# Circuitscape/Circuitscape.jl

Hardware: NVIDIA H100
Metric: pair_solves_per_sec (higher is better)
Workload: dtype f64

## Files before the change

### circuitscape_b200/csrc/cs_b200.cu

```cuda
#include "../../include/cs_b200.h"

#include <cuda_runtime.h>
#include <cub/device/device_radix_sort.cuh>
#include <cub/device/device_scan.cuh>
#include <cub/device/device_select.cuh>

#include <algorithm>
#include <chrono>
#include <cmath>
#include <cstdarg>
#include <cstdio>
#include <cstdlib>
#include <cstring>
#include <limits>
#include <string>
#include <type_traits>
#include <vector>

#include "amg_host.hpp"
#include "win_host.hpp"
#include "kernels.cuh"
#include "raster_assembly.cuh"
#include "setup_device.hpp"

using namespace csb;

namespace {

thread_local std::string g_create_error;

constexpr int PROF_CLASSES = 20;
constexpr int PROF_PJ = 7;
constexpr int PROF_CGF = 8;
constexpr int PROF_RSW = 9;

struct GraphSlot {
  cudaGraphExec_t exec = nullptr;
  int chunk = 0;
  int64_t kernels = 0, spmms = 0;
  cudaGraphExec_t loop_exec = nullptr;
  int64_t loop_kernels = 0, loop_spmms = 0;
};

}

struct DevCsr {
  int* rowptr = nullptr;
  int* colidx = nullptr;
  void* vals = nullptr;
  int* bstart = nullptr;
  int nblocks = 0;
  int nrows = 0;
  int64_t nnz = 0;
  int lpr = 1;
  WinMeta* win_meta = nullptr;
  unsigned char* blob = nullptr;
  int has_dinv = 0;
  int64_t win_blocks = 0;
  int win_nblocks = 0;
  void* dia = nullptr;
  size_t dia_ld = 0;
  int dia_nr = 0;
  int dia_half = 0;
  int* ell_col = nullptr;
  void* ell_val = nullptr;
  size_t ell_ld = 0;
};

struct DevLevel {
  int64_t n = 0, n_pad = 0;
  DevCsr A, P, R;
  void* dinv = nullptr;
  double omega = 2.0 / 3.0;
  void *x = nullptr, *b = nullptr, *t = nullptr, *y = nullptr;
};

struct cs_b200_handle {
  int device = 0;
  int dtype = CS_B200_F64;
  int64_t n = 0, n_pad = 0, nnz = 0;
  int* d_rowptr = nullptr;
  int* d_colidx = nullptr;
  void* d_vals = nullptr;
  bool owns_matrix = true;
  void* d_vals0 = nullptr;
  void* d_fg = nullptr;
  void* d_plan = nullptr;
  int64_t plan_ncol = 0, plan_nset = 0, plan_nsrc = 0;
  void* d_dinv = nullptr;
  int* d_bstart = nullptr;
  int nblocks = 0;
  int ktmax = 8;
  void *X = nullptr, *R = nullptr, *P = nullptr, *AP = nullptr, *B = nullptr, *stage = nullptr;
  void* Z = nullptr;
  void* P2 = nullptr;
  void* R2 = nullptr;
  DevCsr A0;
  std::vector<DevLevel> lv;
  double* d_pinv = nullptr;
  double amg_opc = 0.0;
  bool amg = false;
  bool mixed = false;
  std::vector<DevLevel> lv32;
  void *R32 = nullptr, *X32 = nullptr, *T32 = nullptr, *Z32 = nullptr;
  void *d_cum = nullptr, *d_max = nullptr;
  int* d_bptr = nullptr;
  int64_t nb = 0;
  void* d_cum_branch = nullptr;
  void* d_branch_stage = nullptr;
  PanelCtl* d_ctl = nullptr;
  PanelCtl* h_ctl = nullptr;
  double* d_partials = nullptr;
  float* d_flush = nullptr;
  size_t flush_elems = 0;
  cudaStream_t stream = nullptr;
  cudaEvent_t ev0 = nullptr, ev1 = nullptr, ev2 = nullptr, ev3 = nullptr;
  long long* d_sp_rows = nullptr;
// ... 1229 lines not shown
template <typename F>
decltype(auto) with_width(int kt, F&& f) {
  DISPATCH_KT(kt, return f(std::integral_constant<int, KT>{}));
}

template <typename F>
decltype(auto) with_type_width(const cs_b200_handle* h, int kt, F&& f) {
  return with_type(h, [&](auto t) -> decltype(auto) {
    return with_width(kt, [&](auto KT) -> decltype(auto) { return f(t, KT); });
  });
}

struct ColumnDriver {
  cs_b200_handle* h;
  bool any_fail = false, any_maxit = false;
  std::string msg;

  template <typename Panel>
  int run(int64_t c_begin, int64_t c_end, Panel&& panel) {
    for (int64_t c0 = c_begin; c0 < c_end;) {
      const int kt = next_kt(c_end - c0, h->ktmax);
      if (int rc = with_width(kt, [&](auto KT) { return panel(KT, c0); })) return rc;
      c0 += kt;
    }
    return CS_B200_OK;
  }

  template <typename T, int KT>
  int solve(int64_t c0, double rtol, int64_t itmax, int64_t* iters, double* relres, bool masked = false) {
    h->rg_on = masked;
    const int rc = solve_panel<T, KT>(h, rtol, itmax);
    h->rg_on = false;
    h->pair_b = false;
    if (!rc) gather(KT, c0, iters, relres, itmax);
    return rc;
  }

  void gather(int kt, int64_t c0, int64_t* iters, double* relres, int64_t itmax) {
    for (int c = 0; c < kt; ++c) {
      const PanelCtl& ct = *h->h_ctl;
      const double bn = ct.bnorm[c];
      const double rr = bn > 0 ? std::sqrt(ct.resid[c] / bn) : 0.0;
      if (iters) iters[c0 + c] = ct.iters[c];
      if (relres) relres[c0 + c] = rr;
      h->stats.iterations += ct.iters[c];
      if (!(rr < h->opts.resid_gate)) {
        if (!any_fail) {
          char buf[256];
          snprintf(buf, sizeof buf,
                   "CUDA PCG solver residual %g exceeds tolerance %g for column %lld (%d iterations)",
                   rr, h->opts.resid_gate, (long long)(c0 + c + 1), ct.iters[c]);
          msg = buf;
        }
        any_fail = true;
      }
      if ((ct.iters[c] >= itmax || ct.stalled[c]) && std::sqrt(ct.rho[c]) > ct.tol[c]) any_maxit = true;
    }
  }

  int verdict(int rc) const {
    if (rc) return rc;
    if (any_fail) return set_err(h, CS_B200_ERR_RESIDUAL, "%s", msg.c_str());
    if (any_maxit) return set_err(h, CS_B200_ERR_MAXITER, "itmax reached (or the recurrence stagnated) before rtol");
    return CS_B200_OK;
  }
};

template <int KT>
int cur_grid(cs_b200_handle* h) {
  return (int)std::min<int64_t>(h->grid_spmm, (h->n + (NT / KT) - 1) / (NT / KT));
}

template <typename T, int KT>
void launch_cur_max(cs_b200_handle* h) {
  const int grid = cur_grid<KT>(h);
  if (h->A0.dia)
    k_cur_max_dia<T, KT><<<grid, NT, 0, h->stream>>>(dia_view<T>(h->A0), (const T*)h->X, h->d_ctl, h->d_partials);
  else
    k_cur_max<T, KT><<<grid, NT, 0, h->stream>>>((int)h->n, h->d_rowptr, h->d_colidx, (const T*)h->d_vals,
                                                 (const T*)h->X, h->d_ctl, h->d_partials);
  h->stats.kernel_launches++;
}

template <typename T, int KT>
void launch_currents(cs_b200_handle* h, bool want_curr, int accumulate, const void* fg = nullptr) {
  const int grid = cur_grid<KT>(h);
  launch_cur_max<T, KT>(h);
  if (h->A0.dia) {
    const DiaDev<T> a = dia_view<T>(h->A0);
    k_cur_acc_dia<T, KT><<<grid, NT, 0, h->stream>>>(a, (const T*)h->X, (const T*)fg, h->d_ctl,
                                                     want_curr ? (T*)h->AP : nullptr,
                                                     (T*)h->d_cum, (T*)h->d_max, accumulate, h->opts.log_transform, KT);
  } else {
    k_cur_acc<T, KT><<<grid, NT, 0, h->stream>>>((int)h->n, h->d_rowptr, h->d_colidx, (const T*)h->d_vals,
                                                 (const T*)h->X, (const T*)fg, h->d_ctl,
                                                 want_curr ? (T*)h->AP : nullptr,
                                                 (T*)h->d_cum, (T*)h->d_max, accumulate, h->opts.log_transform, KT);
  }
  h->stats.kernel_launches++;
}

struct ColCtl {
  long long src, dst;
  double weight;
};

inline double col_weight(const double* weight, int64_t c) { return weight ? weight[c] : 1.0; }

template <typename Col>
int upload_ctl(cs_b200_handle* h, int kt, Col&& col) {
  PanelCtl* hc = h->h_ctl;
  std::memset(hc, 0, sizeof(PanelCtl));
  for (int c = 0; c < kt; ++c) {
    const ColCtl v = col(c);
    hc->src[c] = v.src;
    hc->dst[c] = v.dst;
    hc->weight[c] = v.weight;
  }
  CK(h, cudaMemcpyAsync(h->d_ctl, hc, sizeof(PanelCtl), cudaMemcpyHostToDevice, h->stream));
  h->stats.h2d_bytes += sizeof(PanelCtl);
  return CS_B200_OK;
}

int read_ctl(cs_b200_handle* h) {
  CK(h, cudaMemcpyAsync(h->h_ctl, h->d_ctl, sizeof(PanelCtl), cudaMemcpyDeviceToHost, h->stream));
  CK(h, cudaStreamSynchronize(h->stream));
  h->stats.d2h_bytes += sizeof(PanelCtl);
  return CS_B200_OK;
}

int upload_sparse_rhs(cs_b200_handle* h, int kt, const int64_t* ptr, const int64_t* rows, const double* vals) {
  int ent_ptr[MAXKT + 1];
  for (int c = 0; c <= kt; ++c) ent_ptr[c] = (int)(ptr[c] - ptr[0]);
  const size_t nent = (size_t)ent_ptr[kt];
  if (!h->d_sp_ptr || nent > h->sp_cap) {
    cudaFree(h->d_sp_ptr); cudaFree(h->d_sp_rows); cudaFree(h->d_sp_vals);
    h->d_sp_ptr = nullptr; h->d_sp_rows = nullptr; h->d_sp_vals = nullptr;
    h->sp_cap = 0;
    const size_t cap = std::max<size_t>(nent, 1024);
    CK(h, cudaMalloc(&h->d_sp_ptr, (MAXKT + 1) * sizeof(int)));
    CK(h, cudaMalloc(&h->d_sp_rows, cap * sizeof(long long)));
    CK(h, cudaMalloc(&h->d_sp_vals, cap * sizeof(double)));
    h->sp_cap = cap;
  }
  CK(h, h2d(h, h->d_sp_ptr, ent_ptr, (kt + 1) * sizeof(int)));
  CK(h, h2d(h, h->d_sp_rows, rows + ptr[0], nent * sizeof(long long)));
  CK(h, h2d(h, h->d_sp_vals, vals + ptr[0], nent * sizeof(double)));
  h->stats.h2d_bytes += (kt + 1) * sizeof(int) + nent * 16.0;
  return CS_B200_OK;
}

int upload_set_segments(cs_b200_handle* h, int kt, const int64_t* set_ptr, const int64_t* set_rows,
                        const int64_t* set_a, const int64_t* set_b) {
  int seg[2 * MAXKT + 1];
  std::vector<int> rows;
  seg[0] = 0;
  for (int s = 0; s < 2 * kt; ++s) {
    const int64_t* sets = (s & 1) ? set_b : set_a;
    if (sets && sets[s / 2] >= 0)
      for (int64_t e = set_ptr[sets[s / 2]]; e < set_ptr[sets[s / 2] + 1]; ++e) rows.push_back((int)set_rows[e]);
    seg[s + 1] = (int)rows.size();
  }
  if (!h->d_rg_seg || rows.size() > h->rg_cap) {
    CK(h, cudaStreamSynchronize(h->stream));
    drop_graphs(h->rgraphs);
    cudaFree(h->d_rg_seg); cudaFree(h->d_rg_rows);
    h->d_rg_seg = nullptr; h->d_rg_rows = nullptr;
    h->rg_cap = 0;
    const size_t cap = std::max<size_t>(rows.size(), 4096);
    CK(h, cudaMalloc(&h->d_rg_seg, (2 * MAXKT + 1) * sizeof(int)));
// ... 2034 lines not shown
```

### circuitscape_b200/csrc/kernels.cuh

```cuda
#pragma once
#include <cuda_runtime.h>
#include <stdint.h>

namespace csb {

constexpr int NT = 256;
constexpr int NWARP = NT / 32;
constexpr int NNZ_CAP = 2304;
constexpr int MAXKT = 8;

struct PanelCtl {
  double rho[MAXKT];
  double pap[MAXKT];
  double alpha[MAXKT];
  double beta[MAXKT];
  double tol[MAXKT];
  double rho0[MAXKT];
  double resid[MAXKT];
  double bnorm[MAXKT];
  double xsrc[MAXKT];
  double xdst[MAXKT];
  double maxpos[MAXKT];
  double maxneg[MAXKT];
  double weight[MAXKT];
// ... 2216 lines not shown
  const int c = threadIdx.x;
  if (c < KT) {
    const long long s = ctl->src[c], d = ctl->dst[c];
    if (s >= 0 && d >= 0 && s != d) {
      B[(size_t)s * KT + c] = T(-1);
      B[(size_t)d * KT + c] = T(1);
    }
  }
}

template <typename T, int KT>
__global__ void k_pair_extract(const T* X, PanelCtl* ctl) {
  const int c = threadIdx.x;
  if (c < KT) {
    const long long s = ctl->src[c], d = ctl->dst[c];
    ctl->xsrc[c] = s >= 0 ? (double)X[(size_t)s * KT + c] : 0.0;
    ctl->xdst[c] = d >= 0 ? (double)X[(size_t)d * KT + c] : 0.0;
  }
}

template <typename T, int KT>
__global__ void k_sparse_rhs(T* B, const int* __restrict__ ent_ptr, const long long* __restrict__ rows,
                             const double* __restrict__ vals) {
  const int c = threadIdx.x;
  if (c < KT)
    for (int e = ent_ptr[c]; e < ent_ptr[c + 1]; ++e) B[(size_t)rows[e] * KT + c] += (T)vals[e];
}

template <typename T, int KT>
__global__ void k_probe(const T* __restrict__ X, const PanelCtl* __restrict__ ctl,
                        const long long* __restrict__ probe, int nprobe, T* __restrict__ out) {
  for (int e = blockIdx.x * blockDim.x + threadIdx.x; e < nprobe * KT; e += gridDim.x * blockDim.x) {
    const int c = e / nprobe, i = e % nprobe;
    out[e] = (T)((double)X[(size_t)probe[i] * KT + c] - ctl->xsrc[c]);
  }
}

template <typename T, int KT>
__global__ void k_combine(int n, size_t n_pad, const T* __restrict__ U, const int* __restrict__ ci,
                          const int* __restrict__ cj, T* __restrict__ X) {
  const size_t total = n_pad * KT;
  for (size_t e = (size_t)blockIdx.x * blockDim.x + threadIdx.x; e < total; e += (size_t)gridDim.x * blockDim.x) {
    const size_t i = e / KT;
    const int c = (int)(e % KT);
    T v = T(0);
    if (i < (size_t)n) {
      const int a = ci[c], b = cj[c];
      v = (b >= 0 ? U[(size_t)b * n_pad + i] : T(0)) - (a >= 0 ? U[(size_t)a * n_pad + i] : T(0));
    }
    X[e] = v;
  }
}

template <typename T, int KT>
__global__ void k_cm_to_panel(int n, size_t ld, const T* __restrict__ cm, T* __restrict__ panel,
                              int ncols) {
  const size_t total = (size_t)n * KT;
  for (size_t e = (size_t)blockIdx.x * blockDim.x + threadIdx.x; e < total;
       e += (size_t)gridDim.x * blockDim.x) {
    const size_t i = e / KT;
    const int c = (int)(e % KT);
    panel[e] = c < ncols ? cm[(size_t)c * ld + i] : T(0);
  }
}
template <typename T, int KT>
__global__ void k_panel_to_cm(int n, size_t ld, const T* __restrict__ panel, T* __restrict__ cm,
                              const PanelCtl* ctl, int use_shift) {
  const size_t total = (size_t)n * KT;
  for (size_t e = (size_t)blockIdx.x * blockDim.x + threadIdx.x; e < total;
       e += (size_t)gridDim.x * blockDim.x) {
    const size_t i = e / KT;
    const int c = (int)(e % KT);
    const T sh = use_shift ? (T)ctl->xsrc[c] : T(0);
    cm[(size_t)c * ld + i] = panel[e] - sh;
  }
}

template <typename T>
__device__ __forceinline__ void ground_current(T x, T& inflow, T& outflow) {
  if (x < T(0)) inflow -= x;
  if (x > T(0)) outflow += x;
}

template <typename T, int KT>
__global__ void __launch_bounds__(NT)
k_cur_max(int n, const int* __restrict__ rowptr, const int* __restrict__ colidx,
          const T* __restrict__ vals, const T* __restrict__ V, PanelCtl* ctl, double* partials) {
  CSB_REDUCE_SMEM(2, KT)
  const int c = threadIdx.x % KT;
  constexpr int RPP = NT / KT;
  double mp = -1.0e300, mn = -1.0e300;
  for (int row = blockIdx.x * RPP + threadIdx.x / KT; row < n; row += gridDim.x * RPP) {
    const T vi = V[(size_t)row * KT + c];
    for (int j = rowptr[row]; j < rowptr[row + 1]; ++j) {
      const int col = colidx[j];
      if (col > row) {
        const T d = fabs(vals[j]) * (vi - V[(size_t)col * KT + c]);
        mp = fmax(mp, (double)d);
        mn = fmax(mn, (double)(-d));
      }
    }
  }
  double v[2][1] = {{mp}, {mn}};
  if (grid_reduce<KT, 1, 2, true>(v, partials, &ctl->ticket, s_warp, s_tree, s_out)) {
    if (threadIdx.x < KT) {
      ctl->maxpos[threadIdx.x] = s_out[threadIdx.x];
      ctl->maxneg[threadIdx.x] = s_out[KT + threadIdx.x];
    }
  }
}

template <typename T, int KT>
__global__ void __launch_bounds__(NT)
k_cur_acc(int n, const int* __restrict__ rowptr, const int* __restrict__ colidx,
          const T* __restrict__ vals, const T* __restrict__ V, const T* __restrict__ fg, const PanelCtl* ctl,
          T* __restrict__ cur_out , T* __restrict__ cum, T* __restrict__ mx,
          int accumulate, int log_transform, int ncols) {
  const int c = threadIdx.x % KT;
  constexpr int RPP = NT / KT;
  const T maxpos = (T)ctl->maxpos[c], maxneg = (T)ctl->maxneg[c];
  const double w = ctl->weight[c];
  const int nrow_iter = (n + RPP - 1) / RPP;
  for (int it = blockIdx.x; it < nrow_iter; it += gridDim.x) {
    const int row = it * RPP + threadIdx.x / KT;
    T cur = T(0);
    if (row < n) {
      const T vi = V[(size_t)row * KT + c];
      T inflow = T(0), outflow = T(0);
      for (int j = rowptr[row]; j < rowptr[row + 1]; ++j) {
        const int col = colidx[j];
        if (col == row) continue;
        const T d = fabs(vals[j]) * (vi - V[(size_t)col * KT + c]);
        if (!(fabs(d / maxneg) < T(1e-8)) && d > T(0)) outflow += d;
        if (!(fabs(d / maxpos) < T(1e-8)) && d < T(0)) inflow -= d;
      }
      if (fg) ground_current(fg[row] * vi, inflow, outflow);
      cur = inflow > outflow ? inflow : outflow;
      if (cur_out) cur_out[(size_t)row * KT + c] = cur;
    }
    if (accumulate) {
      T val = cur;
      if (log_transform) val = cur > T(0) ? (T)log10((double)cur) : T(-9999);
      const unsigned mask = 0xffffffffu;
      const int lane = threadIdx.x & 31;
      const int base = lane - c;
      double s = 0.0;
      T m = T(-1.0e30);
#pragma unroll
      for (int cc = 0; cc < KT; ++cc) {
        const T vv = __shfl_sync(mask, val, base + cc);
        const double ww = __shfl_sync(mask, w, base + cc);
        if (cc < ncols && ww != 0.0) {
          s += ww * (double)vv;
          m = vv > m ? vv : m;
        }
      }
      if (c == 0 && row < n) {
        cum[row] = (T)((double)cum[row] + s);
        if (mx) mx[row] = m > mx[row] ? m : mx[row];
      }
    }
  }
}

template <typename T, int KT>
__global__ void __launch_bounds__(NT)
k_cur_max_dia(const DiaDev<T> A, const T* __restrict__ V, PanelCtl* ctl, double* partials) {
  CSB_REDUCE_SMEM(2, KT)
  const int c = threadIdx.x % KT;
  constexpr int RPP = NT / KT;
  const int n = A.n, nr = A.nr;
  double mp = -1.0e300, mn = -1.0e300;
  for (int row = blockIdx.x * RPP + threadIdx.x / KT; row < n; row += gridDim.x * RPP) {
    T a[4], vj[4];
    const T vi = V[(size_t)row * KT + c];
#pragma unroll
    for (int q = 0; q < 4; ++q) {
      const int s = 5 + q;
      a[q] = __ldg(A.run(s) + row);
      const int j = min(n - 1, row + (s / 3 - 1) * nr + (s % 3 - 1));
      vj[q] = V[(size_t)j * KT + c];
    }
#pragma unroll
    for (int q = 0; q < 4; ++q)
      if (a[q] != T(0)) {
        const T d = fabs(a[q]) * (vi - vj[q]);
        mp = fmax(mp, (double)d);
        mn = fmax(mn, (double)(-d));
      }
  }
  double v[2][1] = {{mp}, {mn}};
  if (grid_reduce<KT, 1, 2, true>(v, partials, &ctl->ticket, s_warp, s_tree, s_out)) {
    if (threadIdx.x < KT) {
      ctl->maxpos[threadIdx.x] = s_out[threadIdx.x];
      ctl->maxneg[threadIdx.x] = s_out[KT + threadIdx.x];
    }
  }
}

template <typename T, int KT>
__global__ void __launch_bounds__(NT)
k_cur_acc_dia(const DiaDev<T> A, const T* __restrict__ V, const T* __restrict__ fg, const PanelCtl* ctl,
              T* __restrict__ cur_out,
              T* __restrict__ cum, T* __restrict__ mx, int accumulate, int log_transform, int ncols) {
  const int c = threadIdx.x % KT;
  constexpr int RPP = NT / KT;
  const int n = A.n, nr = A.nr;
  const T maxpos = (T)ctl->maxpos[c], maxneg = (T)ctl->maxneg[c];
  const double w = ctl->weight[c];
  const int nrow_iter = (n + RPP - 1) / RPP;
  for (int it = blockIdx.x; it < nrow_iter; it += gridDim.x) {
    const int row = it * RPP + threadIdx.x / KT;
    T cur = T(0);
    if (row < n) {
      T a[9], vj[9];
#pragma unroll
      for (int s = 0; s < 9; ++s) {
        a[s] = A.at(s, row);
        const int j = max(0, min(n - 1, row + (s / 3 - 1) * nr + (s % 3 - 1)));
        vj[s] = V[(size_t)j * KT + c];
      }
      const T vi = vj[4];
      T inflow = T(0), outflow = T(0);
#pragma unroll
      for (int s = 0; s < 9; ++s) {
        if (s == 4) continue;
        const T d = fabs(a[s]) * (vi - vj[s]);
        if (!(fabs(d / maxneg) < T(1e-8)) && d > T(0)) outflow += d;
        if (!(fabs(d / maxpos) < T(1e-8)) && d < T(0)) inflow -= d;
      }
      if (fg) ground_current(fg[row] * vi, inflow, outflow);
      cur = inflow > outflow ? inflow : outflow;
      if (cur_out) cur_out[(size_t)row * KT + c] = cur;
    }
    if (accumulate) {
      T val = cur;
      if (log_transform) val = cur > T(0) ? (T)log10((double)cur) : T(-9999);
      const unsigned mask = 0xffffffffu;
      const int lane = threadIdx.x & 31;
      const int base = lane - c;
      double s = 0.0;
      T m = T(-1.0e30);
#pragma unroll
      for (int cc = 0; cc < KT; ++cc) {
        const T vv = __shfl_sync(mask, val, base + cc);
        const double ww = __shfl_sync(mask, w, base + cc);
        if (cc < ncols && ww != 0.0) {
          s += ww * (double)vv;
          m = vv > m ? vv : m;
        }
      }
      if (c == 0 && row < n) {
        cum[row] = (T)((double)cum[row] + s);
        if (mx) mx[row] = m > mx[row] ? m : mx[row];
      }
    }
  }
}

__global__ void k_branch_count(int n, const int* __restrict__ rowptr, const int* __restrict__ colidx,
                               int* __restrict__ cnt, int* bad_row) {
  for (int row = blockIdx.x * blockDim.x + threadIdx.x; row < n; row += gridDim.x * blockDim.x) {
    int low = 0;
    for (int j = rowptr[row]; j < rowptr[row + 1]; ++j) {
      const int col = colidx[j];
      if (j > rowptr[row] && col <= colidx[j - 1]) atomicMin(bad_row, row);
      low += col < row;
    }
    cnt[row] = low;
  }
}

__global__ void k_branch_ends(int n, const int* __restrict__ rowptr, const int* __restrict__ colidx,
                              const int* __restrict__ bptr, long long* __restrict__ lo, long long* __restrict__ hi) {
  for (int row = blockIdx.x * blockDim.x + threadIdx.x; row < n; row += gridDim.x * blockDim.x)
    for (int e = bptr[row], j = rowptr[row]; e < bptr[row + 1]; ++e, ++j) {
      lo[e] = colidx[j];
      hi[e] = row;
    }
}

template <typename T, int KT>
__global__ void __launch_bounds__(NT)
k_branch_cur(int n, const int* __restrict__ rowptr, const int* __restrict__ colidx, const T* __restrict__ vals,
             const int* __restrict__ bptr, const T* __restrict__ V, const PanelCtl* ctl, T* __restrict__ out,
             size_t ld, T* __restrict__ cum, int ncols) {
  T maxpos[KT];
#pragma unroll
  for (int c = 0; c < KT; ++c) maxpos[c] = (T)ctl->maxpos[c];
  for (int row = blockIdx.x * NT + threadIdx.x; row < n; row += gridDim.x * NT) {
    const int e0 = bptr[row], e1 = bptr[row + 1];
    if (e0 == e1) continue;
    T vhi[KT];
#pragma unroll
    for (int c = 0; c < KT; ++c) vhi[c] = V[(size_t)row * KT + c];
    for (int e = e0, j = rowptr[row]; e < e1; ++e, ++j) {
      const int lo = colidx[j];
      const T a = fabs(vals[j]);
      double s = 0.0;
#pragma unroll
      for (int c = 0; c < KT; ++c) {
        const T d = a * (V[(size_t)lo * KT + c] - vhi[c]);
        const T b = !(fabs(d / maxpos[c]) < T(1e-8)) ? fabs(d) : T(0);
        if (out) out[(size_t)c * ld + e] = b;
        if (cum) {
          const double w = ctl->weight[c];
          if (c < ncols && w != 0.0) s += w * (double)b;
        }
      }
      if (cum) cum[e] = (T)((double)cum[e] + s);
    }
  }
}

template <typename T, int KT>
__global__ void k_owner_sum(int n, const T* __restrict__ X, const long long* __restrict__ owner, long long c0,
                            T* __restrict__ vsum) {
  for (int row = blockIdx.x * blockDim.x + threadIdx.x; row < n; row += gridDim.x * blockDim.x) {
    const long long c = owner[row] - c0;
    if (c >= 0 && c < KT) vsum[row] += X[(size_t)row * KT + c];
  }
}

__global__ void k_set_ctl(PanelCtl* ctl, double rtol, double atol, int itmax, int stall_limit) {
  ctl->stall_limit = stall_limit;
  ctl->rtol = rtol;
  ctl->atol = atol;
  ctl->itmax = itmax;
  ctl->init = 1;
  ctl->iter = 0;
}

__global__ void k_set_stall(PanelCtl* ctl, int stall_limit) { ctl->stall_limit = stall_limit; }

template <typename T>
__global__ void k_fill(T* p, size_t n, T v) {
  for (size_t i = (size_t)blockIdx.x * blockDim.x + threadIdx.x; i < n;
       i += (size_t)gridDim.x * blockDim.x)
    p[i] = v;
}
// ... 359 lines not shown
```

### circuitscape_b200/solver.py

```python
from __future__ import annotations

import ctypes as C
from dataclasses import dataclass

import numpy as np
import scipy.sparse as sp

from . import _lib

CUDAB200 = ["cuda", "gpu", "b200", "cg+jacobi+cuda", "cg+amg+cuda"]


@dataclass
class CUDASolver:
    bs: int = 1000
    precision: str = "double"
    device: int = 0
    rtol: float = 1e-6
    itmax: int = 100_000
    precond: str = "amg"
    panel_width: int = 8
    check_every: int = 16
    use_graph: object = True
    window: str = "auto"
# ... 141 lines not shown
        while True:
            lev = {}
            for name, which in (("A", 0), ("P", 1), ("R", 2)):
                nr, nc, nnz = C.c_int64(), C.c_int64(), C.c_int64()
                om, win = C.c_double(), C.c_int()
                rc = self._lib.cs_b200_level_info(self._h, l, which, C.byref(nr), C.byref(nc), C.byref(nnz),
                                                  C.byref(om), C.byref(win))
                if rc != _lib.OK:
                    lev[name] = None
                    continue
                rp = np.empty(nr.value + 1, dtype=np.int32)
                ci = np.empty(nnz.value, dtype=np.int32)
                va = np.empty(nnz.value, dtype=np.float64)
                _lib.check(self._lib, self._h,
                           self._lib.cs_b200_level_csr(self._h, l, which, _lib._ptr(rp), _lib._ptr(ci), _lib._ptr(va)))
                lev[name] = sp.csr_matrix((va, ci, rp), shape=(nr.value, nc.value))
                lev["omega"] = om.value
                lev[name + "_windowed"] = bool(win.value)
                lev[name + "_stencil"] = win.value == 2
            if lev["A"] is None:
                break
            slots = C.c_int()
            _lib.check(self._lib, self._h, self._lib.cs_b200_level_stencil(self._h, l, C.byref(slots)))
            lev["A_stencil_slots"] = slots.value
            out.append(lev)
            l += 1
        return out

    def set_grounds(self, finite=None, dirichlet=None):
        g = None if finite is None else np.ascontiguousarray(finite, dtype=self.dtype)
        m = None if dirichlet is None else np.ascontiguousarray(np.asarray(dirichlet) != 0, dtype=np.uint8)
        assert g is None or len(g) == self.n
        assert m is None or len(m) == self.n
        _lib.check(self._lib, self._h, self._lib.cs_b200_set_grounds(self._h, _lib._ptr(g), _lib._ptr(m)))

    def operator_form(self):
        win = C.c_int()
        rc = self._lib.cs_b200_level_info(self._h, 0, 0, None, None, None, None, C.byref(win))
        _lib.check(self._lib, self._h, rc)
        return {2: "stencil", 1: "windowed"}.get(win.value, "csr")

    def close(self):
        if getattr(self, "_h", None) is not None and self._h.value:
            self._lib.cs_b200_destroy(self._h)
            self._h = C.c_void_p()

    __del__ = close

    def __enter__(self):
        return self

    def __exit__(self, *a):
        self.close()

    def _limits(self, rtol, itmax):
        return (self.solver.rtol if rtol is None else rtol, self.solver.itmax if itmax is None else itmax)

    def _columns(self, k, want_volt, want_curr):
        cols = lambda want: np.empty((self.n, k), dtype=self.dtype, order="F") if want else None
        return cols(want_volt), cols(want_curr), np.zeros(k, dtype=np.int64), np.zeros(k, dtype=np.float64)

    def _io(self, a):
        return a.astype(self.io_dtype) if a is not None and self.io_dtype != self.dtype else a

    def stats(self):
        st = _lib.Stats()
        self._lib.cs_b200_get_stats(self._h, C.byref(st))
        return st.as_dict()

    def stream_ptr(self):
        p = C.c_void_p()
        _lib.check(self._lib, self._h, self._lib.cs_b200_stream(self._h, C.byref(p)))
        return p.value or 0

    def profile_spmm(self, enable):
        ms, cnt = C.c_double(), C.c_int64()
        _lib.check(self._lib, self._h,
                   self._lib.cs_b200_profile_spmm(self._h, -1 if enable is None else int(bool(enable)),
                                                  C.byref(ms), C.byref(cnt)))
        return ms.value, cnt.value

    def profile_classes(self):
        names = ["plain", "cg", "residual_gate", "residual", "jacobi", "jacobi_dot", "prolong_add", "prolong_jacobi_fused",
                 "cg_step_fused", "residual_sweep_fused"]
        ms = np.zeros(2 * len(names))
        by = np.zeros(2 * len(names))
        ln = np.zeros(2 * len(names), dtype=np.int64)
        _lib.check(self._lib, self._h, self._lib.cs_b200_profile_classes_n(self._h, len(ms), _lib._ptr(ms), _lib._ptr(by),
                                                                           _lib._ptr(ln)))
        return {f"{names[i // 2]}_{'f32' if i % 2 else 'f64'}": (float(ms[i]), float(by[i]), int(ln[i]))
                for i in range(2 * len(names)) if ln[i]}

    def profile_bytes(self):
        b = C.c_double()
        _lib.check(self._lib, self._h, self._lib.cs_b200_profile_bytes(self._h, C.byref(b)))
        return b.value

    def spmv(self, x, reps=1):
        x = np.ascontiguousarray(x, dtype=self.dtype)
        y = np.empty_like(x)
        ms = C.c_double()
        rc = self._lib.cs_b200_spmv(self._h, _lib._ptr(x), _lib._ptr(y), reps, C.byref(ms))
        _lib.check(self._lib, self._h, rc)
        return y, ms.value

    def spmm(self, X):
        X = np.asfortranarray(X, dtype=self.dtype)
        Y = np.empty_like(X, order="F")
        rc = self._lib.cs_b200_spmm(self._h, X.shape[1], _lib._ptr(X), _lib._ptr(Y))
        _lib.check(self._lib, self._h, rc)
        return Y

    def apply_precond(self, R):
        R = np.asarray(R, dtype=self.dtype)
        vec = R.ndim == 1
        X = np.asfortranarray(R.reshape(self.n, -1))
        Z = np.empty_like(X, order="F")
        rz = np.zeros(X.shape[1])
        rc = self._lib.cs_b200_apply_precond(self._h, X.shape[1], _lib._ptr(X), _lib._ptr(Z), _lib._ptr(rz))
        _lib.check(self._lib, self._h, rc)
        return (Z[:, 0] if vec else Z), rz

    def bench_spmm(self, k, reps=20, flush_l2=False):
        ms = C.c_double()
        rc = self._lib.cs_b200_bench_spmm(self._h, k, reps, 1 if flush_l2 else 0, C.byref(ms))
        _lib.check(self._lib, self._h, rc)
        return ms.value

    def bench_cg_iter(self, k, reps=20):
        ms = C.c_double()
        rc = self._lib.cs_b200_bench_cg_iter(self._h, k, reps, C.byref(ms))
        _lib.check(self._lib, self._h, rc)
        return ms.value

    def solve_rhs(self, rhs, rtol=None, itmax=None, raise_on_residual=True, out=None):
        rhs = np.asarray(rhs, dtype=self.dtype)
        vec = rhs.ndim == 1
        b = np.asfortranarray(rhs.reshape(self.n, -1))
        k = b.shape[1]
        x = out if out is not None else np.empty_like(b, order="F")
        assert x.flags.f_contiguous and x.shape == b.shape and x.dtype == b.dtype
        iters = np.zeros(k, dtype=np.int64)
        relres = np.zeros(k, dtype=np.float64)
        rc = self._lib.cs_b200_solve_rhs(self._h, k, _lib._ptr(b), _lib._ptr(x), *self._limits(rtol, itmax),
                                         _lib._ptr(iters), _lib._ptr(relres))
        self._raise(rc, raise_on_residual)
        if out is None:
            x = self._io(x)
        return (x[:, 0] if vec else x), iters, relres

    def solve_pairs(self, src, dst, weight=None, want_volt=False, want_curr=False,
                    accumulate=False, rtol=None, itmax=None, raise_on_residual=True, want_branch=False):
        src = np.ascontiguousarray(src, dtype=np.int64)
        dst = np.ascontiguousarray(dst, dtype=np.int64)
        k = len(src)
        R = np.zeros(k, dtype=self.dtype)
        volt, curr, iters, relres = self._columns(k, want_volt, want_curr)
        args = (self._h, k, _lib._ptr(src), _lib._ptr(dst), _lib._ptr(_opt(weight, np.float64)),
                *self._limits(rtol, itmax), _lib._ptr(R), _lib._ptr(volt), _lib._ptr(curr), 1 if accumulate else 0,
                _lib._ptr(iters), _lib._ptr(relres))
        branch = None
        if want_branch:
            branch = np.empty((self._num_branches(), k), dtype=self.dtype, order="F")
            rc = self._lib.cs_b200_solve_pairs_branch(*args, _lib._ptr(branch))
        else:
            rc = self._lib.cs_b200_solve_pairs(*args)
        self._raise(rc, raise_on_residual)
# ... 285 lines not shown
```

### profiles/run_panel_ends.py

```python
#!/usr/bin/env python
import argparse
import json
import os
import re
import subprocess
import sys
import tempfile
from collections import defaultdict

ROOT = os.path.dirname(os.path.dirname(os.path.abspath(__file__)))
sys.path.insert(0, ROOT)
SWITCH = "CS_B200_NO_FUSED_PANEL_ENDS"


def card():
    try:
        out = subprocess.run(["nvidia-smi", "--query-gpu=name,power.limit", "--format=csv,noheader"],
                             capture_output=True, text=True, timeout=30).stdout.strip().splitlines()
        name, pl = [s.strip() for s in out[0].split(",")]
        return {"name": name, "power_limit": pl}
    except Exception as e:
        return {"name": None, "power_limit": None, "error": str(e)}


def short(name):
    name = name.replace("(anonymous namespace)::", "").replace("csb::", "")
    name = re.sub(r"^void ", "", name)
    depth, cut = 0, len(name)
    for i, ch in enumerate(name):
        if ch == "<":
            depth += 1
        elif ch == ">":
            depth -= 1
        elif ch == "(" and depth == 0 and i > 0:
            cut = i
            break
    return name[:cut].replace(" ", "")


def child(rows, npairs, trace_path):
    import numpy as np
    import torch
    from torch.profiler import ProfilerActivity, profile
    import circuitscape_b200 as cb
    from circuitscape_b200 import graph

    L, _ = graph.synthetic_raster_laplacian(rows, rows, seed=42)
    npts = 2
    while npts * (npts - 1) // 2 < 128:
        npts += 1
    src, dst = graph.all_pairs(graph.focal_nodes(L.shape[0], npts, seed=7), limit=128)
    src, dst = src[:npairs], dst[:npairs]
    with cb.construct_cholesky_factor(L, cb.CUDASolver()) as f:
        f.reset_currents()
        f.solve_pairs(src, dst, accumulate=True)
        torch.cuda.synchronize()
        f.reset_currents()
        with profile(activities=[ProfilerActivity.CUDA]) as prof:
            out = f.solve_pairs(src, dst, accumulate=True)
            torch.cuda.synchronize()
        prof.export_chrome_trace(trace_path)
        np.save(trace_path + ".R.npy", np.asarray(out["R"]))


def panels(trace_path):
    with open(trace_path) as fh:
        ev = json.load(fh)["traceEvents"]
    dev = sorted((e for e in ev if e.get("ph") == "X" and e.get("cat") in ("kernel", "gpu_memset", "gpu_memcpy")),
                 key=lambda e: e["ts"])
    out, cur = [], []
    for e in dev:
        cur.append(e)
        if short(e["name"]).startswith("k_cur_acc_dia"):
            out.append(cur)
            cur = []
    res = []
    for p in out:
        conds = [i for i, e in enumerate(p) if short(e["name"]).startswith("k_loop_cond")]
        if not conds:
            raise SystemExit("no k_loop_cond in a panel: the device WHILE loop did not run")
        start, end = p[:conds[0]], p[conds[-1] + 1:]

        def passes(seg):
            agg = defaultdict(lambda: [0, 0.0])
            for e in seg:
                k = short(e["name"])
                agg[k][0] += 1
                agg[k][1] += e["dur"] / 1000.0
            return [{"pass": k, "launches": n, "ms": round(ms, 4)} for k, (n, ms) in agg.items()]

        res.append({"start_ms": round(sum(e["dur"] for e in start) / 1000.0, 4),
                    "end_ms": round(sum(e["dur"] for e in end) / 1000.0, 4),
                    "loop_cond_kernels": len(conds),
                    "start": passes(start), "end": passes(end)})
    return res


def main():
    ap = argparse.ArgumentParser()
    ap.add_argument("--rows", type=int, default=3163)
    ap.add_argument("--pairs", type=int, default=16)
    ap.add_argument("--out", default=None)
    ap.add_argument("--child", default=None, help=argparse.SUPPRESS)
    a = ap.parse_args()
    if a.child:
        child(a.rows, a.pairs, a.child)
        return
    import numpy as np
    result = {"card": card(), "rows": a.rows, "pairs": a.pairs, "settings": {}}
    with tempfile.TemporaryDirectory() as tmp:
        R = {}
        for name, off in (("on", False), ("off", True)):
            env = dict(os.environ)
            env.pop(SWITCH, None)
            if off:
                env[SWITCH] = "1"
            trace = os.path.join(tmp, f"{name}.json")
            subprocess.run([sys.executable, os.path.abspath(__file__), "--rows", str(a.rows), "--pairs", str(a.pairs),
                            "--child", trace], env=env, check=True, cwd=ROOT)
            ps = panels(trace)
            R[name] = np.load(trace + ".R.npy")
            result["settings"][name] = {
                "start_ms_per_panel": round(sum(p["start_ms"] for p in ps) / len(ps), 4),
                "end_ms_per_panel": round(sum(p["end_ms"] for p in ps) / len(ps), 4),
                "panels": ps}
        result["R_identical"] = bool(np.array_equal(R["on"], R["off"]))
    line = json.dumps(result)
    print(line)
    if a.out:
        with open(a.out, "w") as fh:
            fh.write(line + "\n")


if __name__ == "__main__":
    main()
```

Baseline: 147.7.

## Stream node-current accumulation through shared-memory stencil pipeline

Adds a k_cur_acc_pipe kernel for DIA stencil matrices that stages voltage rows and diagonals through a shared-memory ring using the existing stencil_pipe async-copy scheme, replacing the per-thread gather in k_cur_acc_dia. The relative 1e-8 cutoff test is replaced by precomputed per-column absolute bounds, and the exact division runs only when a value falls in the ambiguous band. The goal is to cut redundant global loads and divisions in the per-panel current pass. The cost is extra shared memory per block and a different launch configuration. An env var can turn it off.

```diff
diff --git a/circuitscape_b200/csrc/cs_b200.cu b/circuitscape_b200/csrc/cs_b200.cu
--- a/circuitscape_b200/csrc/cs_b200.cu
+++ b/circuitscape_b200/csrc/cs_b200.cu
@@ -29,10 +29,11 @@
 
 thread_local std::string g_create_error;
 
-constexpr int PROF_CLASSES = 20;
+constexpr int PROF_CLASSES = 22;
 constexpr int PROF_PJ = 7;
 constexpr int PROF_CGF = 8;
 constexpr int PROF_RSW = 9;
+constexpr int PROF_CUR = 10;
 
 struct GraphSlot {
   cudaGraphExec_t exec = nullptr;
@@ -1428,10 +1429,34 @@
   h->stats.kernel_launches++;
 }
 
+inline bool streamed_currents(const cs_b200_handle* h) {
+  static const bool off = std::getenv("CS_B200_NO_STREAMED_CURRENTS") != nullptr;
+  return !off && h->A0.dia && stencil_pipe();
+}
+
+template <typename T, int KT, bool HALF>
+void launch_cur_acc_pipe(cs_b200_handle* h, const DiaDev<T>& a, const T* fg, T* cur_out, int accumulate) {
+  constexpr int SMEM = StPipe<T, KT, SP_PLAIN, HALF>::D::BYTES;
+  set_max_smem_once<k_cur_acc_pipe<T, KT, HALF>>(h, SMEM);
+  k_cur_acc_pipe<T, KT, HALF><<<stencil_grid<T, KT>(h, h->A0), NT, SMEM, h->stream>>>(
+      a, (const T*)h->X, fg, h->d_ctl, cur_out, (T*)h->d_cum, (T*)h->d_max, accumulate, h->opts.log_transform, KT);
+}
+
 template <typename T, int KT>
 void launch_currents(cs_b200_handle* h, bool want_curr, int accumulate, const void* fg = nullptr) {
   const int grid = cur_grid<KT>(h);
   launch_cur_max<T, KT>(h);
+  if (streamed_currents(h)) {
+    const DiaDev<T> a = dia_view<T>(h->A0);
+    const double rowb = (double)h->n * sizeof(T);
+    const double fb = rowb * KT + rowb * (a.half ? 5 : 9) + (want_curr ? rowb * KT : 0.0) + (fg ? rowb : 0.0) +
+                      (accumulate ? 4.0 * rowb : 0.0);
+    const ProfScope prof(h, true, PROF_CUR, sizeof(T) == 4, fb);
+    T* const cur_out = want_curr ? (T*)h->AP : nullptr;
+    if (a.half) launch_cur_acc_pipe<T, KT, true>(h, a, (const T*)fg, cur_out, accumulate);
+    else launch_cur_acc_pipe<T, KT, false>(h, a, (const T*)fg, cur_out, accumulate);
+    return;
+  }
   if (h->A0.dia) {
     const DiaDev<T> a = dia_view<T>(h->A0);
     k_cur_acc_dia<T, KT><<<grid, NT, 0, h->stream>>>(a, (const T*)h->X, (const T*)fg, h->d_ctl,
diff --git a/circuitscape_b200/csrc/kernels.cuh b/circuitscape_b200/csrc/kernels.cuh
--- a/circuitscape_b200/csrc/kernels.cuh
+++ b/circuitscape_b200/csrc/kernels.cuh
@@ -2322,6 +2322,58 @@
   if (x > T(0)) outflow += x;
 }
 
+template <typename T> struct CurCut {
+  T lo, hi;
+  static constexpr T C = T(1e-8);
+  CurCut() = default;
+  __host__ __device__ __forceinline__ explicit CurCut(T m) {
+    constexpr bool F64 = sizeof(T) == 8;
+    const T DELTA = F64 ? T(0x1p-47) : T(0x1p-18);
+    const T FLOOR = F64 ? T(0x1p-960) : T(0x1p-90);
+    const T am = m < T(0) ? -m : m;
+    if (am >= FLOOR && am <= T(F64 ? 1.7976931348623157e308 : 3.40282347e38f) && m != T(-1.0e300)) {
+      const T cl = C * (T(1) - DELTA), ch = C * (T(1) + DELTA);
+      lo = am * cl;
+      hi = am * ch;
+    } else {
+      lo = T(0);
+      hi = T(INFINITY);
+    }
+  }
+  template <class M> __host__ __device__ __forceinline__ bool keep(T d, M&& m) const {
+    const T ad = d < T(0) ? -d : d;
+    if (ad < lo) return false;
+    if (ad > hi) return true;
+    return !(fabs(d / m()) < C);
+  }
+};
+
+template <typename T>
+__device__ __forceinline__ T cur_map_val(T cur, int log_transform) {
+  return log_transform ? (cur > T(0) ? (T)log10((double)cur) : T(-9999)) : cur;
+}
+
+template <typename T, int KT, class Col>
+__device__ __forceinline__ void cur_accumulate(Col&& col, int ncols, bool write, int row, T* __restrict__ cum,
+                                               T* __restrict__ mx) {
+  double s = 0.0;
+  T m = T(-1.0e30);
+#pragma unroll
+  for (int cc = 0; cc < KT; ++cc) {
+    T vv;
+    double ww;
+    col(cc, vv, ww);
+    if (cc < ncols && ww != 0.0) {
+      s += ww * (double)vv;
+      m = vv > m ? vv : m;
+    }
+  }
+  if (write) {
+    cum[row] = (T)((double)cum[row] + s);
+    if (mx) mx[row] = m > mx[row] ? m : mx[row];
+  }
+}
+
 template <typename T, int KT>
 __global__ void __launch_bounds__(NT)
 k_cur_max(int n, const int* __restrict__ rowptr, const int* __restrict__ colidx,
@@ -2474,28 +2526,134 @@
       if (cur_out) cur_out[(size_t)row * KT + c] = cur;
     }
     if (accumulate) {
-      T val = cur;
-      if (log_transform) val = cur > T(0) ? (T)log10((double)cur) : T(-9999);
-      const unsigned mask = 0xffffffffu;
-      const int lane = threadIdx.x & 31;
-      const int base = lane - c;
-      double s = 0.0;
-      T m = T(-1.0e30);
-#pragma unroll
-      for (int cc = 0; cc < KT; ++cc) {
-        const T vv = __shfl_sync(mask, val, base + cc);
-        const double ww = __shfl_sync(mask, w, base + cc);
-        if (cc < ncols && ww != 0.0) {
-          s += ww * (double)vv;
-          m = vv > m ? vv : m;
+      const T val = cur_map_val(cur, log_transform);
+      const int base = (threadIdx.x & 31) - c;
+      cur_accumulate<T, KT>(
+          [&](int cc, T& vv, double& ww) {
+            vv = __shfl_sync(0xffffffffu, val, base + cc);
+            ww = __shfl_sync(0xffffffffu, w, base + cc);
+          },
+          ncols, c == 0 && row < n, row, cum, mx);
+    }
+  }
+}
+
+template <typename T, int KT> constexpr int cur_pipe_minb() { return sizeof(T) == 8 && KT >= 4 ? 2 : 3; }
+
+template <typename T, int KT, bool HALF>
+__global__ void __launch_bounds__(NT, cur_pipe_minb<T, KT>())
+k_cur_acc_pipe(const DiaDev<T> A, const T* __restrict__ V, const T* __restrict__ fg, const PanelCtl* ctl,
+               T* __restrict__ cur_out, T* __restrict__ cum, T* __restrict__ mx, int accumulate, int log_transform,
+               int ncols) {
+  using SP = StPipe<T, KT, SP_PLAIN, HALF>;
+  constexpr int CPT = SP::CPT, RPP = SP::RPP, S = SP::D::S, CG = KT / CPT;
+  constexpr int RP = S + 3;
+  extern __shared__ __align__(128) unsigned char st_sm[];
+  unsigned char* const pring = st_sm;
+  unsigned char* const oring = st_sm + RP * SP::PANEL;
+  const int tid = threadIdx.x;
+  const int cg = tid % CG, rl = tid / CG, c0 = cg * CPT;
+  const int n = A.n, nr = A.nr;
+  __shared__ CurCut<T> s_cut[2][KT];
+  if (tid < 2 * KT) s_cut[tid / KT][tid % KT] = CurCut<T>((T)(tid < KT ? ctl->maxpos[tid] : ctl->maxneg[tid - KT]));
+
+  auto issue = [&](const StStep& s, int lp, int lo) {
+    unsigned char* ps = pring + lp * SP::PANEL;
+    const long long g0 = (long long)s.c * nr + s.r0 - 1;
+    cp_rows<T, KT, RPP + 2>(reinterpret_cast<T*>(ps), V, g0, n);
+    if (HALF) {
+      int u0, u1;
+      s.half_runs(u0, u1);
+      cp_diag_half<T, RPP>(reinterpret_cast<T*>(ps + SP::PDG), A, g0, u0, u1);
+    } else if (s.c > s.cs) {
+      cp_diag<T, RPP>(reinterpret_cast<T*>(oring + lo * SP::OWN), A, (long long)(s.c - 1) * nr + s.r0);
+    }
+  };
+  auto compute = [&](const StStep& s, int sp, int so) {
+    const int c = s.c - 1, r = s.r0 + rl;
+    const long long row_l = (long long)c * nr + r;
+    const bool live = r < nr && row_l < n;
+    const int row = live ? (int)row_l : 0;
+    T cur[CPT];
+#pragma unroll
+    for (int i = 0; i < CPT; ++i) cur[i] = T(0);
+    if (live) {
+      const T* xs[3];
+      const T* ds[3];
+#pragma unroll
+      for (int d = 0; d < 3; ++d) {
+        const int k = sp + d + RP - 2;
+        const unsigned char* p = pring + (k >= RP ? k - RP : k) * SP::PANEL;
+        xs[d] = reinterpret_cast<const T*>(p);
+        ds[d] = reinterpret_cast<const T*>(p + SP::PDG);
+      }
+      const T* dg = reinterpret_cast<const T*>(oring + so * SP::OWN);
+      T vi[CPT], inflow[CPT], outflow[CPT];
+      ldvec<T, CPT>(xs[1] + (rl + 1) * KT + c0, vi);
+      bool open = false;
+#pragma unroll
+      for (int i = 0; i < CPT; ++i) inflow[i] = outflow[i] = T(0);
+#pragma unroll
+      for (int s9 = 0; s9 < 9; ++s9) {
+        if (s9 == 4) continue;
+        T vj[CPT];
+        ldvec<T, CPT>(xs[s9 / 3] + (rl + s9 % 3) * KT + c0, vj);
+        const T a = fabs(HALF ? st_half_val<T, RPP>(ds, s9, rl) : dg[s9 * RPP + rl]);
+#pragma unroll
+        for (int i = 0; i < CPT; ++i) {
+          const T d = a * (vi[i] - vj[i]);
+          const bool pos = d > T(0), neg = d < T(0);
+          const CurCut<T>& cut = s_cut[pos ? 1 : 0][c0 + i];
+          const T ad = fabs(d);
+          const bool keep = ad > cut.hi;
+          open |= (pos || neg) && !keep && !(ad < cut.lo);
+          outflow[i] += pos && keep ? d : T(0);
+          inflow[i] -= neg && keep ? d : T(0);
         }
       }
-      if (c == 0 && row < n) {
-        cum[row] = (T)((double)cum[row] + s);
-        if (mx) mx[row] = m > mx[row] ? m : mx[row];
-      }
-    }
-  }
+      if (open) {
+#pragma unroll
+        for (int i = 0; i < CPT; ++i) inflow[i] = outflow[i] = T(0);
+#pragma unroll 1
+        for (int s9 = 0; s9 < 9; ++s9) {
+          if (s9 == 4) continue;
+          const int d3 = s9 / 3;
+          const T* const x3 = d3 == 0 ? xs[0] : d3 == 1 ? xs[1] : xs[2];
+          T vj[CPT];
+          ldvec<T, CPT>(x3 + (rl + s9 % 3) * KT + c0, vj);
+          const T a = fabs(!HALF ? dg[s9 * RPP + rl]
+                           : s9 < 4 ? (d3 == 0 ? ds[0] : ds[1])[(4 - s9) * (RPP + 2) + rl + s9 % 3]
+                                    : ds[1][(s9 - 4) * (RPP + 2) + rl + 1]);
+#pragma unroll
+          for (int i = 0; i < CPT; ++i) {
+            const T d = a * (vi[i] - vj[i]);
+            if (d > T(0) && s_cut[1][c0 + i].keep(d, [&] { return (T)ctl->maxneg[c0 + i]; })) outflow[i] += d;
+            if (d < T(0) && s_cut[0][c0 + i].keep(d, [&] { return (T)ctl->maxpos[c0 + i]; })) inflow[i] -= d;
+          }
+        }
+      }
+      const T g = fg ? fg[row] : T(0);
+#pragma unroll
+      for (int i = 0; i < CPT; ++i) {
+        if (fg) ground_current(g * vi[i], inflow[i], outflow[i]);
+        cur[i] = inflow[i] > outflow[i] ? inflow[i] : outflow[i];
+      }
+      if (cur_out) stvec<T, CPT>(cur_out + (size_t)row * KT + c0, cur);
+    }
+    if (accumulate) {
+      T val[CPT];
+#pragma unroll
+      for (int i = 0; i < CPT; ++i) val[i] = cur_map_val(cur[i], log_transform);
+      const int base = (tid & 31) - cg;
+      cur_accumulate<T, KT>(
+          [&](int cc, T& vv, double& ww) {
+            vv = CG == 1 ? val[cc % CPT] : __shfl_sync(0xffffffffu, val[cc % CPT], base + cc / CPT);
+            ww = ctl->weight[cc];
+          },
+          ncols, cg == 0 && live, row, cum, mx);
+    }
+  };
+  stencil_pipe<S, RPP>(n, nr, issue, compute);
 }
 
 __global__ void k_branch_count(int n, const int* __restrict__ rowptr, const int* __restrict__ colidx,
diff --git a/circuitscape_b200/solver.py b/circuitscape_b200/solver.py
--- a/circuitscape_b200/solver.py
+++ b/circuitscape_b200/solver.py
@@ -247,7 +247,7 @@
 
     def profile_classes(self):
         names = ["plain", "cg", "residual_gate", "residual", "jacobi", "jacobi_dot", "prolong_add", "prolong_jacobi_fused",
-                 "cg_step_fused", "residual_sweep_fused"]
+                 "cg_step_fused", "residual_sweep_fused", "node_currents"]
         ms = np.zeros(2 * len(names))
         by = np.zeros(2 * len(names))
         ln = np.zeros(2 * len(names), dtype=np.int64)
diff --git a/profiles/run_panel_ends.py b/profiles/run_panel_ends.py
--- a/profiles/run_panel_ends.py
+++ b/profiles/run_panel_ends.py
@@ -10,7 +10,8 @@
 
 ROOT = os.path.dirname(os.path.dirname(os.path.abspath(__file__)))
 sys.path.insert(0, ROOT)
-SWITCH = "CS_B200_NO_FUSED_PANEL_ENDS"
+SETTINGS = {"on": (), "ends_off": ("CS_B200_NO_FUSED_PANEL_ENDS",), "currents_off": ("CS_B200_NO_STREAMED_CURRENTS",)}
+CUR_PASSES = ("k_cur_acc_pipe", "k_cur_acc_dia")
 
 
 def card():
@@ -71,7 +72,7 @@
     out, cur = [], []
     for e in dev:
         cur.append(e)
-        if short(e["name"]).startswith("k_cur_acc_dia"):
+        if short(e["name"]).startswith(CUR_PASSES):
             out.append(cur)
             cur = []
     res = []
@@ -110,11 +111,11 @@
     result = {"card": card(), "rows": a.rows, "pairs": a.pairs, "settings": {}}
     with tempfile.TemporaryDirectory() as tmp:
         R = {}
-        for name, off in (("on", False), ("off", True)):
+        for name, off in SETTINGS.items():
             env = dict(os.environ)
-            env.pop(SWITCH, None)
-            if off:
-                env[SWITCH] = "1"
+            for sw in (v for vs in SETTINGS.values() for v in vs):
+                env.pop(sw, None)
+            env.update({sw: "1" for sw in off})
             trace = os.path.join(tmp, f"{name}.json")
             subprocess.run([sys.executable, os.path.abspath(__file__), "--rows", str(a.rows), "--pairs", str(a.pairs),
                             "--child", trace], env=env, check=True, cwd=ROOT)
@@ -124,7 +125,7 @@
                 "start_ms_per_panel": round(sum(p["start_ms"] for p in ps) / len(ps), 4),
                 "end_ms_per_panel": round(sum(p["end_ms"] for p in ps) / len(ps), 4),
                 "panels": ps}
-        result["R_identical"] = bool(np.array_equal(R["on"], R["off"]))
+        result["R_identical"] = all(bool(np.array_equal(R["on"], R[k])) for k in R)
     line = json.dumps(result)
     print(line)
     if a.out:
```

Result: faster. 150.8 (median of 6 runs) (+2.1%).
